# liyheng/MAGPO

Hardware: AMD Instinct MI355X
Metric: env-steps/sec (all agents stepping jointly), CoordSum-4ag, full MAGPO update loop (higher is better)
Workload: dtype f32 (fp32 MFMA; as bf16 x3 operand splits = 24 mantissa bits, six products, fp32 accumulate: the GRU forward scan's recurrent GEMM)

## Files before the change

magpo_amd/csrc/gru.hip:

```cpp
#include "common.hpp"
#include <stdlib.h>

namespace magpo {

constexpr int H = 128;
constexpr int HP = H + LDP;
constexpr int G3 = 3 * H;
constexpr int G3P = G3 + LDP;

struct GruArgs {
  const float* xi;
  const float* Wht;
  const float* b_hn;
  const float* h0;
  const int* h0_idx;
  const unsigned char* reset;
  float* hs;
  float* gates;
  float* hprev;
  int T, A, NR;
  int time_major;
  float* h_last;
  const int* xi_cls;
};

#ifdef MAGPO_GRU_PROF
__device__ unsigned long long g_gru_prof[8];
#define GP_DECL() unsigned long long gp_acc[8] = {0, 0, 0, 0, 0, 0, 0, 0}; unsigned long long gp_last = clock64();
#define GP(k) do { unsigned long long t_ = clock64(); gp_acc[k] += t_ - gp_last; gp_last = t_; } while (0)
#define GP_FLUSH() do { if (threadIdx.x == 0 && (blockIdx.x & 63) == 0) { for (int k_ = 0; k_ < 8; ++k_) atomicAdd(&g_gru_prof[k_], gp_acc[k_]); } } while (0)
#else
#define GP_DECL()
#define GP(k)
#define GP_FLUSH()
#endif

__device__ __forceinline__ long tok_row(int rho, int t, int T, int A) {
  int seq = rho / A, ag = rho - seq * A;
  return ((long)seq * T + t) * A + ag;
}

template <bool FULL, int MODE, int ROWS>
__global__ __launch_bounds__(256, 1) void k_gru_scan_fwd(GruArgs a, int block0) {
  constexpr bool TM = MODE == 1;
  __shared__ __align__(16) float hbuf[2][ROWS * HP];
  extern __shared__ unsigned char rflag[];
  const int tid = threadIdx.x, lane = tid & 63, wave = tid >> 6, lr = lane & 31, h = lane >> 5;
  const int rho0 = (block0 + blockIdx.x) * ROWS;
  const int col = 32 * wave + lr;
  const int T = a.T;
  float4 wf[3][16];
#pragma unroll
  for (int g = 0; g < 3; ++g)
#pragma unroll
    for (int u = 0; u < 16; ++u) wf[g][u] = *reinterpret_cast<const float4*>(a.Wht + ((long)g * H + col) * H + 64 * h + 4 * u);
  const float bhn = a.b_hn[col];
  for (int i = tid; i < ROWS * T; i += 256) {
    const int rl = i / T, t = i - rl * T;
    const int rho = min(rho0 + rl, a.NR - 1);
    rflag[i] = TM ? a.reset[(long)t * (a.NR / a.A) + rho / a.A] : a.reset[(long)(rho / a.A) * T + t];
  }
  int* ctab = reinterpret_cast<int*>(rflag + ROWS * T);
  const bool by_cls = a.xi_cls != nullptr;
  if (by_cls) {
    for (int i = tid; i < ROWS * T; i += 256) {
      const int rl = i / T, t = i - rl * T;
      const int rho = min(rho0 + rl, a.NR - 1);
      ctab[i] = a.xi_cls[TM ? (long)t * a.NR + rho : tok_row(rho, t, T, a.A)];
    }
  }
  for (int i = tid; i < ROWS * (H / 4); i += 256) {
    int r = i / (H / 4), c4 = i - r * (H / 4);
    int rho = rho0 + r;
    float4 v = make_float4(0.f, 0.f, 0.f, 0.f);
    if (rho < a.NR) {
      int seq = rho / a.A;
      if (!(TM ? a.reset[seq] : a.reset[(long)seq * T])) {
        long src = a.h0_idx ? a.h0_idx[rho] : rho;
        v = *reinterpret_cast<const float4*>(a.h0 + src * H + 4 * c4);
      }
    }
    *reinterpret_cast<float4*>(&hbuf[0][r * HP + 4 * c4]) = v;
  }
  __shared__ long rbase[ROWS];
  if (tid < ROWS) rbase[tid] = TM ? (long)min(rho0 + tid, a.NR - 1) : tok_row(min(rho0 + tid, a.NR - 1), 0, T, a.A);
  const long t_stride = TM ? a.NR : a.A;
  __syncthreads();
  GP_DECL();
  for (int t = 0; t < T; ++t) {
    const float* hold = hbuf[t & 1];
    float* hnew = hbuf[(t + 1) & 1];
#pragma unroll
    for (int wr = 0; wr < ROWS / 32; ++wr) {
      GP(6);
      float xr[16], xz[16], xn[16];
      long rowi[16];
#pragma unroll
      for (int i = 0; i < 16; ++i) {
        const int rl = 32 * wr + (i & 3) + 8 * (i >> 2) + 4 * h;
        const long row = rbase[rl] + (long)t * t_stride;
        rowi[i] = row;
        const float* x = a.xi + (by_cls ? (long)ctab[rl * T + t] : row) * G3;
        xr[i] = x[col]; xz[i] = x[H + col]; xn[i] = x[2 * H + col];
      }
      float hpv[16];
      unsigned char rf[16];
      const int tn = t + 1 < T ? t + 1 : t;
#pragma unroll
      for (int i = 0; i < 16; ++i) {
        const int rl = 32 * wr + (i & 3) + 8 * (i >> 2) + 4 * h;
        hpv[i] = hold[rl * HP + col];
        rf[i] = rflag[rl * T + tn];
      }
      GP(0 + 3 * wr);
      f32x16 ar, az, an;
#pragma unroll
      for (int i = 0; i < 16; ++i) { ar[i] = 0.f; az[i] = 0.f; an[i] = 0.f; }
      const float* ap = hold + (32 * wr + lr) * HP + 64 * h;
#pragma unroll
      for (int u = 0; u < 16; ++u) {
        const float4 av = *reinterpret_cast<const float4*>(ap + 4 * u);
        ar = __builtin_amdgcn_mfma_f32_32x32x2f32(av.x, wf[0][u].x, ar, 0, 0, 0);
        az = __builtin_amdgcn_mfma_f32_32x32x2f32(av.x, wf[1][u].x, az, 0, 0, 0);
        an = __builtin_amdgcn_mfma_f32_32x32x2f32(av.x, wf[2][u].x, an, 0, 0, 0);
        ar = __builtin_amdgcn_mfma_f32_32x32x2f32(av.y, wf[0][u].y, ar, 0, 0, 0);
        az = __builtin_amdgcn_mfma_f32_32x32x2f32(av.y, wf[1][u].y, az, 0, 0, 0);
        an = __builtin_amdgcn_mfma_f32_32x32x2f32(av.y, wf[2][u].y, an, 0, 0, 0);
        ar = __builtin_amdgcn_mfma_f32_32x32x2f32(av.z, wf[0][u].z, ar, 0, 0, 0);
        az = __builtin_amdgcn_mfma_f32_32x32x2f32(av.z, wf[1][u].z, az, 0, 0, 0);
        an = __builtin_amdgcn_mfma_f32_32x32x2f32(av.z, wf[2][u].z, an, 0, 0, 0);
        ar = __builtin_amdgcn_mfma_f32_32x32x2f32(av.w, wf[0][u].w, ar, 0, 0, 0);
        az = __builtin_amdgcn_mfma_f32_32x32x2f32(av.w, wf[1][u].w, az, 0, 0, 0);
        an = __builtin_amdgcn_mfma_f32_32x32x2f32(av.w, wf[2][u].w, an, 0, 0, 0);
      }
      GP(1 + 3 * wr);
      const bool more = t + 1 < T;
#pragma unroll
      for (int i = 0; i < 16; ++i) {
        const int rl = 32 * wr + (i & 3) + 8 * (i >> 2) + 4 * h;
        const long row = rowi[i];
        const float hb = an[i] + bhn;
        const float r = fast_sigmoid(xr[i] + ar[i]);
        const float z = fast_sigmoid(xz[i] + az[i]);
        const float n = fast_tanh(xn[i] + r * hb);
        const float hp = hpv[i];
        float hn_new = (1.0f - z) * n + z * hp;
        if (FULL || rho0 + rl < a.NR) {
          if (MODE == 0) {
            a.hs[row * H + col] = hn_new;
            *reinterpret_cast<float4*>(a.gates + row * (4 * H) + 4 * col) = make_float4(r, z, n, hb);
            a.hprev[row * H + col] = hp;
          } else if (MODE == 1) {
            if (!more) a.h_last[(long)(rho0 + rl) * H + col] = hn_new;
          } else {
            if (a.hs) a.hs[row * H + col] = hn_new;
            if (a.gates) {
              *reinterpret_cast<float4*>(a.gates + row * (4 * H) + 4 * col) = make_float4(r, z, n, hb);
            }
            if (a.hprev) a.hprev[row * H + col] = hp;
          }
        }
        hnew[rl * HP + col] = (more & (rf[i] != 0)) ? 0.f : hn_new;
      }
      GP(2 + 3 * wr);
    }
    __syncthreads();
    GP(7);
  }
  GP_FLUSH();
}

constexpr int HB = H + 8;

__device__ __forceinline__ void split_bf16(float x, __bf16& hi, __bf16& lo) {
  hi = (__bf16)x;
  lo = (__bf16)(x - (float)hi);
}

template <bool FULL, int NP>
__global__ __launch_bounds__(256, 1) void k_gru_scan_fwd_bf3(GruArgs a, int block0) {
  constexpr int ROWS = NP == 3 ? 32 : 64;
  __shared__ __align__(16) float hf[ROWS * HP];
  __shared__ __align__(16) __bf16 hsp[2][NP][ROWS * HB];
  extern __shared__ unsigned char rflag[];
  const int tid = threadIdx.x, lane = tid & 63, wave = tid >> 6, lr = lane & 31, h = lane >> 5;
  const int rho0 = (block0 + blockIdx.x) * ROWS;
  const int col = 32 * wave + lr;
  const int T = a.T;
  bf16x8 wp[NP][3][8];
#pragma unroll
  for (int g = 0; g < 3; ++g)
#pragma unroll
    for (int s8 = 0; s8 < 8; ++s8) {
      const float* w = a.Wht + ((long)g * H + col) * H + 64 * h + 8 * s8;
      const float4 w0 = *reinterpret_cast<const float4*>(w), w1 = *reinterpret_cast<const float4*>(w + 4);
      const float wv[8] = {w0.x, w0.y, w0.z, w0.w, w1.x, w1.y, w1.z, w1.w};
#pragma unroll
      for (int j = 0; j < 8; ++j) {
        __bf16 pc[NP];
        split_pieces<NP>(wv[j], pc);
#pragma unroll
        for (int q = 0; q < NP; ++q) wp[q][g][s8][j] = pc[q];
      }
    }
  const float bhn = a.b_hn[col];
  for (int i = tid; i < ROWS * T; i += 256) {
    const int rl = i / T, t = i - rl * T;
    const int rho = min(rho0 + rl, a.NR - 1);
    rflag[i] = a.reset[(long)(rho / a.A) * T + t];
  }
  int* ctab = reinterpret_cast<int*>(rflag + ROWS * T);
  const bool by_cls = a.xi_cls != nullptr;
  if (by_cls) {
    for (int i = tid; i < ROWS * T; i += 256) {
      const int rl = i / T, t = i - rl * T;
      ctab[i] = a.xi_cls[tok_row(min(rho0 + rl, a.NR - 1), t, T, a.A)];
    }
  }
  for (int i = tid; i < ROWS * (H / 4); i += 256) {
    const int r = i / (H / 4), c4 = i - r * (H / 4);
    const int rho = rho0 + r;
    float4 v = make_float4(0.f, 0.f, 0.f, 0.f);
    if (rho < a.NR && !a.reset[(long)(rho / a.A) * T]) {
      const long src = a.h0_idx ? a.h0_idx[rho] : rho;
      v = *reinterpret_cast<const float4*>(a.h0 + src * H + 4 * c4);
    }
    *reinterpret_cast<float4*>(&hf[r * HP + 4 * c4]) = v;
    const float vv[4] = {v.x, v.y, v.z, v.w};
#pragma unroll
    for (int j = 0; j < 4; ++j) {
      __bf16 pc[NP];
      split_pieces<NP>(vv[j], pc);
#pragma unroll
      for (int q = 0; q < NP; ++q) hsp[0][q][r * HB + 4 * c4 + j] = pc[q];
    }
  }
  __shared__ long rbase[ROWS];
  if (tid < ROWS) rbase[tid] = tok_row(min(rho0 + tid, a.NR - 1), 0, T, a.A);
  __syncthreads();
  for (int t = 0; t < T; ++t) {
    const int cur = t & 1, nxt = (t + 1) & 1;
#pragma unroll
// ... 533 lines not shown
```

magpo_amd/csrc/linear.hip:

```cpp
#include "common.hpp"
#include <stdlib.h>

namespace magpo {

enum { ACT_NONE = 0, ACT_RELU = 1, ACT_GELU = 2, ACT_SWISH = 3, ACT_MASKPOS = 4, ACT_TANH = 5, ACT_TANHBWD = 6 };

enum { PRO_EMBED_ACT = 1, PRO_EMBED_OBS = 2, PRO_RESNORM = 3, PRO_HEADMID = 4 };
struct ProArgs {
  const float* a; long lda;
  const float* y; long ldy_;
  const float* s1; const float* s2;
  const float* pe; const int* pos; long pos_stride; int npos; int use_pe;
  const float* W; const int* idx; long idx_stride;
  const float* s_obs; int F;
  float* out; long ldout;
  float* outpe; long ldoutpe;
};

__device__ __forceinline__ float half_row_mean_sq(const float4* v) {
  float s = 0.f;
#pragma unroll
  for (int u = 0; u < 8; ++u) s += v[u].x * v[u].x + v[u].y * v[u].y + v[u].z * v[u].z + v[u].w * v[u].w;
  s += __shfl_xor(s, 32, 64);
  return s * (1.0f / 64.0f);
// ... 364 lines not shown
  const bool do_bias = bias_slab != nullptr && kb == 0;
  const bool full_cols = (c0 + 64 * NB <= NOUT) && ((ldy & 3) == 0);

  WP_DECL();
  if (full_cols) {
    float4 nx[4 + 4 * NB];
    constexpr int YR = 16 * NB;
    const int rx = tid >> 4, cx = 4 * (tid & 15);
    const int ry = tid / YR, cy = 4 * (tid % YR);
    const float* xb = X + kb * 64 + cx;
    const float* yb = dY + c0 + cy;
#define WG_LOADX(J, ROW0) nx[J] = *reinterpret_cast<const float4*>(xb + (long)min((int)(ROW0) + rx + 16 * (J), R - 1) * ldx)
#define WG_LOADY(J, ROW0) nx[4 + (J)] = *reinterpret_cast<const float4*>(yb + (long)min((int)(ROW0) + ry + (256 / YR) * (J), R - 1) * ldy)
    {
      const long row0 = (long)min(g, ntiles - 1) * 64;
#pragma unroll
      for (int j = 0; j < 4; ++j) WG_LOADX(j, row0);
#pragma unroll
      for (int j = 0; j < 4 * NB; ++j) WG_LOADY(j, row0);
    }
    for (int tile = g; tile < ntiles; tile += G) {
      const long row0 = (long)tile * 64;
      const long row0n = (long)min(tile + G, ntiles - 1) * 64;
      __syncthreads();
      WP(0);
#pragma unroll
      for (int j = 0; j < 4; ++j) {
        float4 v = nx[j];
        const bool ok = row0 + rx + 16 * j < R;
        v.x = ok ? v.x : 0.f; v.y = ok ? v.y : 0.f; v.z = ok ? v.z : 0.f; v.w = ok ? v.w : 0.f;
        *reinterpret_cast<float4*>(&xs[(rx + 16 * j) * LDX + cx]) = v;
      }
#pragma unroll
      for (int j = 0; j < 4 * NB; ++j) {
        float4 v = nx[4 + j];
        const bool ok = row0 + ry + (256 / YR) * j < R;
        v.x = ok ? v.x : 0.f; v.y = ok ? v.y : 0.f; v.z = ok ? v.z : 0.f; v.w = ok ? v.w : 0.f;
        *reinterpret_cast<float4*>(&ys[(ry + (256 / YR) * j) * LDY + cy]) = v;
      }
      __syncthreads();
      WP(1);
      WP(2);
#pragma unroll
      for (int s = 0; s < 32; ++s) {
        const int tok = 32 * h + s;
        const float a = xs[tok * LDX + 32 * wr + lr];
#pragma unroll
        for (int b = 0; b < NB; ++b) {
          const float bb = ys[tok * LDY + 64 * b + 32 * wc + lr];
          acc[b] = __builtin_amdgcn_mfma_f32_32x32x2f32(a, bb, acc[b], 0, 0, 0);
        }
        if ((s & 1) && (s >> 1) < 4 + 4 * NB) {
          const int li = s >> 1;
          const float* src = li < 4 ? xb + min(row0n + rx + 16 * li, (long)R - 1) * (long)ldx
                                    : yb + min(row0n + ry + (256 / YR) * (li - 4), (long)R - 1) * (long)ldy;
          nx[li] = *reinterpret_cast<const float4*>(src);
        }
      }
      WP(3);
      if (do_bias && tid < 64 * NB) {
        float sb = 0.f;
#pragma unroll 8
        for (int r = 0; r < 64; ++r) sb += ys[r * LDY + tid];
        bsum += sb;
      }
    }
#undef WG_LOADX
#undef WG_LOADY
  } else {
    float4 xq[4], yq[4 * NB];
    auto fetch = [&](int tile) {
      const long row0 = (long)tile * 64;
  #pragma unroll
      for (int j = 0; j < 4; ++j) {
        const int i = tid + 256 * j;
        const int r = i >> 4, c4 = i & 15;
        const long gr = row0 + r;
        xq[j] = make_float4(0.f, 0.f, 0.f, 0.f);
        if (gr < R) xq[j] = *reinterpret_cast<const float4*>(X + gr * (long)ldx + kb * 64 + 4 * c4);
      }
  #pragma unroll
      for (int j = 0; j < 4 * NB; ++j) {
        const int i = tid + 256 * j;
        const int r = i / (16 * NB), c4 = i - r * (16 * NB);
        const long gr = row0 + r;
        const int col = c0 + 4 * c4;
        float4 v = make_float4(0.f, 0.f, 0.f, 0.f);
        if (gr < R) {
          const float* p = dY + gr * (long)ldy + col;
          if (full_cols || col + 3 < NOUT) v = *reinterpret_cast<const float4*>(p);
          else {
            if (col + 0 < NOUT) v.x = p[0];
            if (col + 1 < NOUT) v.y = p[1];
            if (col + 2 < NOUT) v.z = p[2];
          }
        }
        yq[j] = v;
      }
    };
    auto stash = [&]() {
  #pragma unroll
      for (int j = 0; j < 4; ++j) {
        const int i = tid + 256 * j;
        *reinterpret_cast<float4*>(&xs[(i >> 4) * LDX + 4 * (i & 15)]) = xq[j];
      }
  #pragma unroll
      for (int j = 0; j < 4 * NB; ++j) {
        const int i = tid + 256 * j;
        const int r = i / (16 * NB), c4 = i - r * (16 * NB);
        *reinterpret_cast<float4*>(&ys[r * LDY + 4 * c4]) = yq[j];
      }
    };

    if (g < ntiles) fetch(g);
    for (int tile = g; tile < ntiles; tile += G) {
      __syncthreads();
      stash();
      __syncthreads();
      if (tile + G < ntiles) fetch(tile + G);
#pragma unroll 4
      for (int s = 0; s < 32; ++s) {
        const int tok = 32 * h + s;
        const float a = xs[tok * LDX + 32 * wr + lr];
#pragma unroll
        for (int b = 0; b < NB; ++b) {
          const float bb = ys[tok * LDY + 64 * b + 32 * wc + lr];
          acc[b] = __builtin_amdgcn_mfma_f32_32x32x2f32(a, bb, acc[b], 0, 0, 0);
        }
      }
      if (do_bias && tid < 64 * NB) {
        float sb = 0.f;
#pragma unroll 8
        for (int r = 0; r < 64; ++r) sb += ys[r * LDY + tid];
        bsum += sb;
      }
    }
  }
  WP_FLUSH();
  float* out = slab + (long)g * KIN * NOUT;
#pragma unroll
  for (int b = 0; b < NB; ++b) {
    const int n = c0 + 64 * b + 32 * wc + lr;
    if (n < NOUT) {
#pragma unroll
      for (int i = 0; i < 16; ++i) {
        int kr = kb * 64 + 32 * wr + (i & 3) + 8 * (i >> 2) + 4 * h;
        out[(long)kr * NOUT + n] = acc[b][i];
      }
    }
  }
  if (do_bias && tid < 64 * NB && c0 + tid < NOUT) bias_slab[(long)g * NOUT + c0 + tid] = bsum;
}

__global__ __launch_bounds__(1024) void k_reduce_slabs(const float* __restrict__ slab, float* __restrict__ out, int G, long P, long stride,
                                                       float scale, int accumulate) {
  __shared__ float sh[16][64];
  const int tx = threadIdx.x & 63, ty = threadIdx.x >> 6;
  const long p = (long)blockIdx.x * 64 + tx;
  float s0 = 0.f, s1 = 0.f, s2 = 0.f, s3 = 0.f;
  if (p < P) {
    int g = ty;
    for (; g + 48 < G; g += 64) {
      s0 += slab[(long)g * stride + p];
      s1 += slab[(long)(g + 16) * stride + p];
      s2 += slab[(long)(g + 32) * stride + p];
      s3 += slab[(long)(g + 48) * stride + p];
    }
    for (; g < G; g += 16) s0 += slab[(long)g * stride + p];
  }
  sh[ty][tx] = (s0 + s1) + (s2 + s3);
  __syncthreads();
  if (ty == 0 && p < P) {
    float s = 0.f;
#pragma unroll
    for (int i = 0; i < 16; ++i) s += sh[i][tx];
    s *= scale;
    out[p] = accumulate ? out[p] + s : s;
  }
}

__global__ void k_transpose_pad(const float* __restrict__ W, float* __restrict__ Wt, int K, int N, int Npad) {
  int i = blockIdx.x * blockDim.x + threadIdx.x;
  if (i >= Npad * K) return;
  int n = i / K, k = i - n * K;
  Wt[i] = n < N ? W[(long)k * N + n] : 0.f;
}

template <int KT, int NT>
__global__ __launch_bounds__(256, 1) void k_wgrad_full(const float* __restrict__ X, int ldx, const float* __restrict__ dY, int ldy,
                                                       int R, float* __restrict__ slab, float* __restrict__ bias_slab) {
  constexpr int KIN = 32 * KT, NOUT = 128 * NT, LDX = KIN + LDP, LDY = NOUT + LDP;
  constexpr int NX = 64 * KIN / 4 / 256, NY = 64 * NOUT / 4 / 256;
  extern __shared__ __align__(16) float wf_smem[];
  float* xs = wf_smem;
  float* ys = xs + 64 * LDX;
  const int tid = threadIdx.x, lane = tid & 63, wave = tid >> 6, lr = lane & 31, h = lane >> 5;
  const int g = blockIdx.x, G = gridDim.x;
  const int ntiles = (R + 63) >> 6;
  f32x16 acc[KT][NT];
#pragma unroll
  for (int kt = 0; kt < KT; ++kt)
#pragma unroll
    for (int nt = 0; nt < NT; ++nt)
#pragma unroll
      for (int i = 0; i < 16; ++i) acc[kt][nt][i] = 0.f;
  float bsum[(NOUT + 255) / 256];
#pragma unroll
  for (int j = 0; j < (NOUT + 255) / 256; ++j) bsum[j] = 0.f;
  float4 nx[NX + NY];
#define WF_SRC(LI, ROW0)                                                                                                    \
  ((LI) < NX ? X + min((ROW0) + (tid + 256 * (LI)) / (KIN / 4), (long)R - 1) * (long)ldx + 4 * ((tid + 256 * (LI)) % (KIN / 4)) \
             : dY + min((ROW0) + (tid + 256 * ((LI) - NX)) / (NOUT / 4), (long)R - 1) * (long)ldy + 4 * ((tid + 256 * ((LI) - NX)) % (NOUT / 4)))
  {
    const long row0 = (long)min(g, ntiles - 1) * 64;
#pragma unroll
    for (int li = 0; li < NX + NY; ++li) nx[li] = *reinterpret_cast<const float4*>(WF_SRC(li, row0));
  }
  for (int tile = g; tile < ntiles; tile += G) {
    const long row0 = (long)tile * 64;
    const long row0n = (long)min(tile + G, ntiles - 1) * 64;
    __syncthreads();
#pragma unroll
    for (int li = 0; li < NX + NY; ++li) {
      float4 v = nx[li];
      const int idx = tid + 256 * (li < NX ? li : li - NX);
      const int r = li < NX ? idx / (KIN / 4) : idx / (NOUT / 4);
      const int c = li < NX ? 4 * (idx % (KIN / 4)) : 4 * (idx % (NOUT / 4));
      const bool ok = row0 + r < R;
      v.x = ok ? v.x : 0.f; v.y = ok ? v.y : 0.f; v.z = ok ? v.z : 0.f; v.w = ok ? v.w : 0.f;
      if (li < NX) *reinterpret_cast<float4*>(&xs[r * LDX + c]) = v;
      else *reinterpret_cast<float4*>(&ys[r * LDY + c]) = v;
    }
    __syncthreads();
#pragma unroll
    for (int s = 0; s < 32; ++s) {
      const int tok = 32 * h + s;
      float av[KT], bv[NT];
#pragma unroll
      for (int kt = 0; kt < KT; ++kt) av[kt] = xs[tok * LDX + 32 * kt + lr];
#pragma unroll
      for (int nt = 0; nt < NT; ++nt) bv[nt] = ys[tok * LDY + 32 * NT * wave + 32 * nt + lr];
#pragma unroll
      for (int kt = 0; kt < KT; ++kt)
#pragma unroll
        for (int nt = 0; nt < NT; ++nt) acc[kt][nt] = __builtin_amdgcn_mfma_f32_32x32x2f32(av[kt], bv[nt], acc[kt][nt], 0, 0, 0);
#pragma unroll
      for (int li = 0; li < NX + NY; ++li)
        if (li * 32 / (NX + NY) == s) nx[li] = *reinterpret_cast<const float4*>(WF_SRC(li, row0n));
    }
    if (bias_slab) {
#pragma unroll
      for (int j = 0; j < (NOUT + 255) / 256; ++j) {
        const int col = tid + 256 * j;
        if (col < NOUT) {
          float sb = 0.f;
#pragma unroll 8
          for (int r = 0; r < 64; ++r) sb += ys[r * LDY + col];
          bsum[j] += sb;
        }
      }
    }
  }
#undef WF_SRC
  float* out = slab + (long)g * KIN * NOUT;
#pragma unroll
  for (int kt = 0; kt < KT; ++kt)
#pragma unroll
    for (int nt = 0; nt < NT; ++nt) {
      const int n = 32 * NT * wave + 32 * nt + lr;
#pragma unroll
      for (int i = 0; i < 16; ++i) out[(long)(32 * kt + (i & 3) + 8 * (i >> 2) + 4 * h) * NOUT + n] = acc[kt][nt][i];
    }
  if (bias_slab) {
#pragma unroll
    for (int j = 0; j < (NOUT + 255) / 256; ++j) {
      const int col = tid + 256 * j;
      if (col < NOUT) bias_slab[(long)g * NOUT + col] = bsum[j];
    }
  }
}

__device__ __forceinline__ void split8(const float (&v)[8], bf16x8 (&p)[3]) {
#pragma unroll
  for (int j = 0; j < 8; ++j) {
    __bf16 pc[3];
    split_pieces<3>(v[j], pc);
    p[0][j] = pc[0]; p[1][j] = pc[1]; p[2][j] = pc[2];
  }
}
template <int KT, int NT, int PAD = LDP, bool BF3 = false>
__global__ __launch_bounds__(256, 1) void k_wgrad_full_x(const float* __restrict__ X, int ldx, const float* __restrict__ dY, int ldy,
                                                         int R, float* __restrict__ slab, float* __restrict__ bias_slab) {
  constexpr int KIN = 32 * KT, NOUT = 128 * NT, LDX = KIN + PAD, LDY = NOUT + PAD;
  constexpr int TX = KIN / 4, RPX = 256 / TX, NX = 64 / RPX;
  constexpr int NY = 8 * NT;
  extern __shared__ __align__(16) float wf_smem[];
  float* xs = wf_smem;
  float* ys = xs + 64 * LDX;
  const int tid = threadIdx.x, lane = tid & 63, wave = tid >> 6, lr = lane & 31, h = lane >> 5;
  const int g = blockIdx.x, G = gridDim.x;
  const int ntiles = R >> 6;
  f32x16 acc[KT][NT];
#pragma unroll
  for (int kt = 0; kt < KT; ++kt)
#pragma unroll
    for (int nt = 0; nt < NT; ++nt)
#pragma unroll
      for (int i = 0; i < 16; ++i) acc[kt][nt][i] = 0.f;
  float4 bsum[NT];
#pragma unroll
  for (int j = 0; j < NT; ++j) bsum[j] = make_float4(0.f, 0.f, 0.f, 0.f);
  const unsigned xoff = (unsigned)(tid / TX) * (unsigned)ldx + 4u * (unsigned)(tid % TX);
  const unsigned yoff = (unsigned)(tid >> 5) * (unsigned)ldy + 4u * (unsigned)(tid & 31);
  float* xsw = xs + (tid / TX) * LDX + 4 * (tid % TX);
  float* ysw = ys + (tid >> 5) * LDY + 4 * (tid & 31);
  float4 nxx[NX], nxy[NY];
#define WFX_LOADX(LI, ROW0) nxx[LI] = *reinterpret_cast<const float4*>(X + ((ROW0) + (LI) * RPX) * (long)ldx + xoff)
#define WFX_LOADY(LI, ROW0) nxy[LI] = *reinterpret_cast<const float4*>(dY + ((ROW0) + 8 * ((LI) / NT)) * (long)ldy + 128 * ((LI) % NT) + yoff)
  {
    const long row0 = (long)min(g, ntiles - 1) * 64;
#pragma unroll
    for (int li = 0; li < NX; ++li) { WFX_LOADX(li, row0); }
#pragma unroll
    for (int li = 0; li < NY; ++li) { WFX_LOADY(li, row0); }
  }
  const float* xr = xs + (32 * h) * LDX + lr;
  const float* yr = ys + (32 * h) * LDY + 32 * NT * wave + lr;
  for (int tile = g; tile < ntiles; tile += G) {
    const long row0n = (long)min(tile + G, ntiles - 1) * 64;
    __syncthreads();
#pragma unroll
    for (int li = 0; li < NX; ++li) {
// ... 345 lines not shown
        const float4 a4 = *reinterpret_cast<const float4*>(ard + 4 * u);
        float4 w4;
        if constexpr (WL) w4 = *reinterpret_cast<const float4*>(wrd + 4 * u);
        else w4 = wf[j][u];
        accx = __builtin_amdgcn_mfma_f32_32x32x2f32(a4.x, w4.x, accx, 0, 0, 0);
        accx = __builtin_amdgcn_mfma_f32_32x32x2f32(a4.y, w4.y, accx, 0, 0, 0);
        accx = __builtin_amdgcn_mfma_f32_32x32x2f32(a4.z, w4.z, accx, 0, 0, 0);
        accx = __builtin_amdgcn_mfma_f32_32x32x2f32(a4.w, w4.w, accx, 0, 0, 0);
      }
      const int cb = 32 * (KT * wb + j);
      float* dxt = dX + row0 * lddx + 32 * j;
      const float* mt = MASK == 1 ? aux + row0 * ldaux + 32 * j : nullptr;
#define DB_TR(I) (((I) & 3) + 8 * ((I) >> 2))
      if (full) {
        if constexpr (MASK != 0) {
          float mk[16];
#pragma unroll
          for (int i = 0; i < 16; ++i) mk[i] = MASK == 2 ? xs[(32 * wa + DB_TR(i) + 4 * h) * LDX + cb + lr] : (mt + DB_TR(i) * ldaux)[mo];
#pragma unroll
          for (int i = 0; i < 16; ++i) (dxt + DB_TR(i) * lddx)[so] = mk[i] > 0.f ? accx[i] : 0.f;
        } else {
#pragma unroll
          for (int i = 0; i < 16; ++i) (dxt + DB_TR(i) * lddx)[so] = accx[i];
        }
      } else {
#pragma unroll
        for (int i = 0; i < 16; ++i) {
          if (32 * wa + DB_TR(i) + 4 * h < rleft) {
            float v = accx[i];
            if constexpr (MASK != 0) v = (MASK == 2 ? xs[(32 * wa + DB_TR(i) + 4 * h) * LDX + cb + lr] : (mt + DB_TR(i) * ldaux)[mo]) > 0.f ? v : 0.f;
            (dxt + DB_TR(i) * lddx)[so] = v;
          }
        }
      }
#undef DB_TR
    }
  }
#undef DB_LOADX
#undef DB_LOADY
  if (dwa) {
    const int n = 32 * cbw + lr;
    float* out = slab + (long)g * KIN * NOUT;
    if (n < NOUT) {
#pragma unroll
      for (int kt = 0; kt < KW; ++kt)
#pragma unroll
        for (int i = 0; i < 16; ++i) out[(long)(32 * (kb0 + kt) + (i & 3) + 8 * (i >> 2) + 4 * h) * NOUT + n] = accw[kt][i];
    }
  }
  if (do_bias && bt < NOUT) bias_slab[(long)g * NOUT + bt] = bsum;
}

}

using namespace magpo;

template <auto K>
static auto with_lds(size_t lds) {
  static bool done = false;
  if (!done && lds > 65536) {
    hipFuncSetAttribute(reinterpret_cast<const void*>(K), hipFuncAttributeMaxDynamicSharedMemorySize, (int)lds);
    done = true;
  }
  return K;
}

extern "C" int magpo_linear(const float* X, int ldx, const float* Wt, const float* bias, float* Y, int ldy, float* mask,
                            long R, int KIN, int NOUT, int act, int variant, hipStream_t stream) {
  if (R <= 0) return MAGPO_OK;
  if ((ldx & 3) || NOUT <= 0) { set_error("magpo_linear: ldx must be a multiple of 4, NOUT positive"); return MAGPO_EINVAL; }
  if (KIN != 64 && KIN != 128 && KIN != 192 && KIN != 256 && KIN != 384) { set_error("magpo_linear: KIN must be in {64, 128, 192, 256, 384}"); return MAGPO_EINVAL; }
  if (variant != 0 && variant != 4) { set_error("magpo_linear: variant must be 0 or 4"); return MAGPO_EINVAL; }
  if (act < ACT_NONE || act > ACT_TANHBWD) { set_error("magpo_linear: act must be in [0, 6]"); return MAGPO_EINVAL; }
  const bool needs_mask = act == ACT_MASKPOS || act == ACT_TANHBWD;
  if (needs_mask && !mask) { set_error("magpo_linear: act 4 / 6 (backward masks) need the mask tensor"); return MAGPO_EINVAL; }
  if (!needs_mask && mask) { set_error("magpo_linear: the pre-activation output was removed; the seventh argument is the mask input of act 4 / 6 and must be null otherwise"); return MAGPO_EINVAL; }
  const int ncg = (NOUT + 31) / 32;
  const int nw = (ncg % 4 == 0) ? 4 : 2;
  const int gy = (ncg + nw - 1) / nw;
  const long ntiles = (R + 31) / 32;
  long wk2 = 2048 / nw;
  if (gy >= 3) wk2 /= 2;
  if (wk2 > ntiles) wk2 = ntiles;
  const bool bf3 = variant == 4 && (KIN == 128 || KIN == 192) && nw == 4;
  const size_t lds = bf3 ? (size_t)2 * 3 * 32 * (KIN + 8) * sizeof(__bf16) : (size_t)2 * 32 * (KIN + LDP) * sizeof(float);
  decltype(&k_linear_lds<64, 4>) k;
  if (bf3) k = KIN == 128 ? with_lds<k_linear_lds<128, 4, true>>(lds) : with_lds<k_linear_lds<192, 4, true>>(lds);
  else if (KIN == 64) k = nw == 4 ? with_lds<k_linear_lds<64, 4>>(lds) : with_lds<k_linear_lds<64, 2>>(lds);
  else if (KIN == 128) k = nw == 4 ? with_lds<k_linear_lds<128, 4>>(lds) : with_lds<k_linear_lds<128, 2>>(lds);
  else if (KIN == 192) k = nw == 4 ? with_lds<k_linear_lds<192, 4>>(lds) : with_lds<k_linear_lds<192, 2>>(lds);
  else if (KIN == 256) k = nw == 4 ? with_lds<k_linear_lds<256, 4>>(lds) : with_lds<k_linear_lds<256, 2>>(lds);
  else k = nw == 4 ? with_lds<k_linear_lds<384, 4>>(lds) : with_lds<k_linear_lds<384, 2>>(lds);
  hipLaunchKernelGGL(k, dim3((unsigned)wk2, (unsigned)gy), dim3(64 * nw), lds, stream, X, ldx, Wt, bias, Y, ldy, (int)R, NOUT, act, (const float*)mask);
  return check_launch("magpo_linear");
}

extern "C" int magpo_linear_pro(int pro, const float* a, long lda, const float* y, long ldy_in, const float* s1, const float* s2,
                                const float* pe, const int* pos, long pos_stride, int npos, int use_pe, const float* W,
                                const int* idx, long idx_stride, const float* s_obs, int F, float* out, long ldout,
                                float* outpe, long ldoutpe, const float* Wt, const float* bias, float* Y, long ldy, long R,
                                int NOUT, hipStream_t stream) {
  if (R <= 0) return MAGPO_OK;
  if (pro < 1 || pro > 4 || NOUT <= 0) { set_error("magpo_linear_pro: bad prologue id / NOUT"); return MAGPO_EINVAL; }
  ProArgs p{a, lda, y, ldy_in, s1, s2, pe, pos, pos_stride, npos, use_pe, W, idx, idx_stride, s_obs, F, out, ldout, outpe, ldoutpe};
  const int ncg = (NOUT + 63) / 64;
  const int wpb = ncg < 4 ? ncg : 4;
  const long ntiles = (R + 31) / 32;
  long walkers = 2048 / wpb;
  if (walkers > ntiles) walkers = ntiles;
  dim3 grid((unsigned)walkers, (unsigned)((ncg + 3) / 4)), block(64 * wpb);
#define LP(P_) hipLaunchKernelGGL((k_linear_pro<P_, 2>), grid, block, 0, stream, p, Wt, bias, Y, ldy, (int)R, NOUT)
  switch (pro) {
    case PRO_EMBED_ACT: LP(PRO_EMBED_ACT); break;
    case PRO_EMBED_OBS: LP(PRO_EMBED_OBS); break;
    case PRO_RESNORM: LP(PRO_RESNORM); break;
    default: LP(PRO_HEADMID); break;
  }
#undef LP
  return check_launch("magpo_linear_pro");
}

extern "C" long magpo_wgrad_workspace_floats(int KIN, int NOUT, int G) { return (long)G * ((long)KIN * NOUT + NOUT); }

extern "C" int magpo_wgrad(const float* X, int ldx, const float* dY, int ldy, long R, int KIN, int krows, int NOUT, float* dW,
                           float* db, float* workspace, int G, float scale, int accumulate, int variant, hipStream_t stream) {
  if ((ldx & 3) || (ldy & 3) || KIN % 64) { set_error("magpo_wgrad: bad strides / KIN"); return MAGPO_EINVAL; }
  if (variant != 0 && variant != 64) { set_error("magpo_wgrad: variant must be 0 or 64"); return MAGPO_EINVAL; }
  const bool exact = R % 64 == 0, big = R >= 64 * 256;
  const size_t lds_full = (size_t)64 * (KIN + NOUT) * sizeof(float), lds_pad = (size_t)64 * ((KIN + LDP) + (NOUT + LDP)) * sizeof(float);
  auto bias_slab = [&] { return db ? workspace + (long)G * KIN * NOUT : nullptr; };
  if (big && exact && KIN == 64 && NOUT == 256) {
    if (G > 512) G = 512;
    auto k = with_lds<k_wgrad_full_x<2, 2, 0>>(lds_full);
    hipLaunchKernelGGL(k, dim3(G), dim3(256), lds_full, stream, X, ldx, dY, ldy, (int)R, workspace, bias_slab());
  } else if (big && exact && ((KIN == 64 && NOUT == 192) || (KIN == 128 && NOUT == 128))) {
    if (G > 512) G = 512;
    auto k = KIN == 64 ? with_lds<k_wgrad_full_g<1, 3>>(lds_full) : with_lds<k_wgrad_full_g<2, 2>>(lds_full);
    hipLaunchKernelGGL(k, dim3(G, 1), dim3(256), lds_full, stream, X, ldx, dY, ldy, (int)R, NOUT, workspace, bias_slab());
  } else if (big && KIN == 128 && NOUT == 384) {
    if (G > 256) G = 256;
    auto k = !exact ? with_lds<k_wgrad_full<4, 3>>(lds_pad)
                    : variant == 64 ? with_lds<k_wgrad_full_x<4, 3, LDP, true>>(lds_pad) : with_lds<k_wgrad_full_x<4, 3>>(lds_pad);
    hipLaunchKernelGGL(k, dim3(G), dim3(256), lds_pad, stream, X, ldx, dY, ldy, (int)R, workspace, bias_slab());
  } else {
    const int nb = NOUT >= 128 ? 2 : 1;
    const int per_g = ((NOUT + 64 * nb - 1) / (64 * nb)) * (KIN / 64);
    int g_fit = 256 * (nb == 2 ? 3 : 4) / per_g;
    if (g_fit < 1) g_fit = 1;
    if (G > g_fit) G = g_fit;
    dim3 grid(G, (NOUT + 64 * nb - 1) / (64 * nb), KIN / 64);
    hipLaunchKernelGGL(nb == 2 ? k_wgrad<2> : k_wgrad<1>, grid, dim3(256), 0, stream, X, ldx, dY, ldy, (int)R, KIN, NOUT, workspace, bias_slab());
  }
  const long P = (long)krows * NOUT;
  hipLaunchKernelGGL(k_reduce_slabs, dim3((unsigned)((P + 63) / 64)), dim3(1024), 0, stream, workspace, dW, G, P, (long)KIN * NOUT, scale, accumulate);
  if (db) hipLaunchKernelGGL(k_reduce_slabs, dim3((NOUT + 63) / 64), dim3(1024), 0, stream, bias_slab(), db, G, (long)NOUT, (long)NOUT, scale, accumulate);
  return check_launch("magpo_wgrad");
}

extern "C" int magpo_dense_bwd(const float* X, int ldx, const float* dY, int ldy, const float* W, const float* mask, int ldmask,
                               float* dX, int lddx, long R, int KIN, int NOUT, float* dW, float* db, float* workspace, int G, int act,
                               hipStream_t stream) {
  if (KIN != 64 && KIN != 128) { set_error("magpo_dense_bwd: KIN must be 64 or 128"); return MAGPO_EINVAL; }
  if (NOUT < 1 || NOUT > 64) { set_error("magpo_dense_bwd: NOUT must be in [1, 64]"); return MAGPO_EINVAL; }
  if ((ldx & 3) || (ldy & 3) || (lddx & 3) || ldx < KIN || lddx < KIN || ldy < NOUT) {
    set_error("magpo_dense_bwd: ldx, ldy, lddx must be multiples of 4 and cover KIN / NOUT / KIN columns"); return MAGPO_EINVAL;
  }
  if (act != ACT_NONE && act != ACT_MASKPOS) { set_error("magpo_dense_bwd: act must be 0 or 4"); return MAGPO_EINVAL; }
  if (act == ACT_MASKPOS && !mask) { set_error("magpo_dense_bwd: act 4 needs the mask tensor"); return MAGPO_EINVAL; }
  if (act == ACT_NONE && mask) { set_error("magpo_dense_bwd: the mask argument must be null for act 0"); return MAGPO_EINVAL; }
  if (mask && ((ldmask & 3) || ldmask < KIN)) { set_error("magpo_dense_bwd: ldmask must be a multiple of 4 and cover KIN columns"); return MAGPO_EINVAL; }
  if (R < 1 || R > 0x7fffffffL - 64 || G < 1) { set_error("magpo_dense_bwd: R must be in [1, 2^31 - 65], G positive"); return MAGPO_EINVAL; }
  if (((uintptr_t)X | (uintptr_t)dY) & 15) { set_error("magpo_dense_bwd: X and dY must be 16-byte aligned"); return MAGPO_EINVAL; }
  if (G > 512) G = 512;
  if (G > (R + 63) / 64) G = (int)((R + 63) / 64);
  float* bias_slab = db ? workspace + (long)G * KIN * NOUT : nullptr;
  const int m = act != ACT_MASKPOS ? 0 : (mask == X && ldmask == ldx) ? 2 : 1;
  const bool k2 = KIN == 128, n2 = NOUT > 32;
  decltype(&k_dense_bwd<1, 1, 0>) k;
#define DB_PICK(KT_, NT_) (m == 0 ? k_dense_bwd<KT_, NT_, 0> : m == 1 ? k_dense_bwd<KT_, NT_, 1> : k_dense_bwd<KT_, NT_, 2>)
  if (!k2 && !n2) k = DB_PICK(1, 1);
  else if (!k2) k = DB_PICK(1, 2);
  else if (!n2) k = DB_PICK(2, 1);
  else k = DB_PICK(2, 2);
#undef DB_PICK
  hipLaunchKernelGGL(k, dim3(G), dim3(256), 0, stream, X, ldx, dY, ldy, W, mask, ldmask, dX, lddx, (int)R, NOUT, workspace, bias_slab);
  const long P = (long)KIN * NOUT;
  hipLaunchKernelGGL(k_reduce_slabs, dim3((unsigned)((P + 63) / 64)), dim3(1024), 0, stream, workspace, dW, G, P, P, 1.0f, 0);
  if (db) hipLaunchKernelGGL(k_reduce_slabs, dim3(1), dim3(1024), 0, stream, bias_slab, db, G, (long)NOUT, (long)NOUT, 1.0f, 0);
  return check_launch("magpo_dense_bwd");
}

extern "C" int magpo_reduce_slabs(const float* slab, float* out, int G, long P, long stride, float scale, int accumulate, hipStream_t stream) {
  hipLaunchKernelGGL(k_reduce_slabs, dim3((unsigned)((P + 63) / 64)), dim3(1024), 0, stream, slab, out, G, P, stride, scale, accumulate);
  return check_launch("magpo_reduce_slabs");
}

extern "C" int magpo_transpose_pad(const float* W, float* Wt, int K, int N, int Npad, hipStream_t stream) {
  int total = Npad * K;
  hipLaunchKernelGGL(k_transpose_pad, dim3((total + 255) / 256), dim3(256), 0, stream, W, Wt, K, N, Npad);
  return check_launch("magpo_transpose_pad");
}

#ifdef MAGPO_WG_PROF
extern "C" int magpo_debug_wg_prof(unsigned long long* out_host, int reset) {
  if (hipMemcpyFromSymbol(out_host, HIP_SYMBOL(magpo::g_wg_prof), sizeof(unsigned long long) * 8) != hipSuccess) return MAGPO_ELAUNCH;
  if (reset) { unsigned long long z[8] = {0}; if (hipMemcpyToSymbol(HIP_SYMBOL(magpo::g_wg_prof), z, sizeof(z)) != hipSuccess) return MAGPO_ELAUNCH; }
  return MAGPO_OK;
}
#endif
```

Measured before the change: 4.232 million.

## Skip GRU scan steps before last reset; batch slab reductions into one launch

```diff
diff --git a/magpo_amd/csrc/gru.hip b/magpo_amd/csrc/gru.hip
--- a/magpo_amd/csrc/gru.hip
+++ b/magpo_amd/csrc/gru.hip
@@ -55,10 +55,19 @@
 #pragma unroll
     for (int u = 0; u < 16; ++u) wf[g][u] = *reinterpret_cast<const float4*>(a.Wht + ((long)g * H + col) * H + 64 * h + 4 * u);
   const float bhn = a.b_hn[col];
+  __shared__ __align__(16) int last[TM ? ROWS : 4];
+  if constexpr (TM) {
+    if (tid < ROWS) last[tid] = 0;
+    __syncthreads();
+  }
   for (int i = tid; i < ROWS * T; i += 256) {
     const int rl = i / T, t = i - rl * T;
     const int rho = min(rho0 + rl, a.NR - 1);
-    rflag[i] = TM ? a.reset[(long)t * (a.NR / a.A) + rho / a.A] : a.reset[(long)(rho / a.A) * T + t];
+    const unsigned char f = TM ? a.reset[(long)t * (a.NR / a.A) + rho / a.A] : a.reset[(long)(rho / a.A) * T + t];
+    rflag[i] = f;
+    if constexpr (TM) {
+      if (f && t > 0) atomicMax(&last[rl], t);
+    }
   }
   int* ctab = reinterpret_cast<int*>(rflag + ROWS * T);
   const bool by_cls = a.xi_cls != nullptr;
@@ -69,25 +78,36 @@
       ctab[i] = a.xi_cls[TM ? (long)t * a.NR + rho : tok_row(rho, t, T, a.A)];
     }
   }
+  int t0 = 0;
+  if constexpr (TM) {
+    __syncthreads();
+    int m = T;
+#pragma unroll
+    for (int r4 = 0; r4 < ROWS / 4; ++r4) {
+      const int4 l4 = *reinterpret_cast<const int4*>(&last[4 * r4]);
+      m = min(min(m, min(l4.x, l4.y)), min(l4.z, l4.w));
+    }
+    t0 = __builtin_amdgcn_readfirstlane(m);
+  }
   for (int i = tid; i < ROWS * (H / 4); i += 256) {
     int r = i / (H / 4), c4 = i - r * (H / 4);
     int rho = rho0 + r;
     float4 v = make_float4(0.f, 0.f, 0.f, 0.f);
-    if (rho < a.NR) {
+    if (rho < a.NR && t0 == 0) {
       int seq = rho / a.A;
       if (!(TM ? a.reset[seq] : a.reset[(long)seq * T])) {
         long src = a.h0_idx ? a.h0_idx[rho] : rho;
         v = *reinterpret_cast<const float4*>(a.h0 + src * H + 4 * c4);
       }
     }
-    *reinterpret_cast<float4*>(&hbuf[0][r * HP + 4 * c4]) = v;
+    *reinterpret_cast<float4*>(&hbuf[t0 & 1][r * HP + 4 * c4]) = v;
   }
   __shared__ long rbase[ROWS];
   if (tid < ROWS) rbase[tid] = TM ? (long)min(rho0 + tid, a.NR - 1) : tok_row(min(rho0 + tid, a.NR - 1), 0, T, a.A);
   const long t_stride = TM ? a.NR : a.A;
   __syncthreads();
   GP_DECL();
-  for (int t = 0; t < T; ++t) {
+  for (int t = t0; t < T; ++t) {
     const float* hold = hbuf[t & 1];
     float* hnew = hbuf[(t + 1) & 1];
 #pragma unroll
diff --git a/magpo_amd/csrc/linear.hip b/magpo_amd/csrc/linear.hip
--- a/magpo_amd/csrc/linear.hip
+++ b/magpo_amd/csrc/linear.hip
@@ -540,14 +540,26 @@
   if (do_bias && tid < 64 * NB && c0 + tid < NOUT) bias_slab[(long)g * NOUT + c0 + tid] = bsum;
 }
 
-__global__ __launch_bounds__(1024) void k_reduce_slabs(const float* __restrict__ slab, float* __restrict__ out, int G, long P, long stride,
-                                                       float scale, int accumulate) {
+__device__ __forceinline__ void fold_block(const float* __restrict__ slab, float* __restrict__ out, int G, long P, long stride, float scale,
+                                           int accumulate, long block) {
   __shared__ float sh[16][64];
   const int tx = threadIdx.x & 63, ty = threadIdx.x >> 6;
-  const long p = (long)blockIdx.x * 64 + tx;
+  const long p = block * 64 + tx;
   float s0 = 0.f, s1 = 0.f, s2 = 0.f, s3 = 0.f;
   if (p < P) {
     int g = ty;
+    for (; g + 240 < G; g += 256) {
+      float v[16];
+#pragma unroll
+      for (int k = 0; k < 16; ++k) v[k] = slab[(long)(g + 16 * k) * stride + p];
+#pragma unroll
+      for (int k = 0; k < 16; k += 4) {
+        s0 += v[k];
+        s1 += v[k + 1];
+        s2 += v[k + 2];
+        s3 += v[k + 3];
+      }
+    }
     for (; g + 48 < G; g += 64) {
       s0 += slab[(long)g * stride + p];
       s1 += slab[(long)(g + 16) * stride + p];
@@ -566,6 +578,51 @@
     out[p] = accumulate ? out[p] + s : s;
   }
 }
+
+__global__ __launch_bounds__(1024) void k_reduce_slabs(const float* __restrict__ slab, float* __restrict__ out, int G, long P, long stride,
+                                                       float scale, int accumulate) {
+  fold_block(slab, out, G, P, stride, scale, accumulate, blockIdx.x);
+}
+
+struct FoldJob {
+  const float* slab;
+  float* out;
+  long P, stride;
+  int G, accumulate;
+  float scale;
+};
+struct FoldJobs {
+  FoldJob job[4];
+  unsigned first[5];
+};
+
+__global__ __launch_bounds__(1024) void k_reduce_slabs_multi(FoldJobs t) {
+  const unsigned b = blockIdx.x;
+  const int j = (b >= t.first[1]) + (b >= t.first[2]) + (b >= t.first[3]);
+  const FoldJob& f = t.job[j];
+  fold_block(f.slab, f.out, f.G, f.P, f.stride, f.scale, f.accumulate, b - t.first[j]);
+}
+
+struct FoldLaunch {
+  FoldJobs t{};
+  int n = 0;
+  void add(const float* slab, float* out, int G, long P, long stride, float scale, int accumulate) {
+    if (P <= 0) return;
+    t.job[n] = FoldJob{slab, out, P, stride, G, accumulate, scale};
+    t.first[n + 1] = t.first[n] + (unsigned)((P + 63) / 64);
+    ++n;
+  }
+  void launch(hipStream_t stream) {
+    if (n == 0) return;
+    if (n == 1) {
+      const FoldJob& f = t.job[0];
+      hipLaunchKernelGGL(k_reduce_slabs, dim3(t.first[1]), dim3(1024), 0, stream, f.slab, f.out, f.G, f.P, f.stride, f.scale, f.accumulate);
+      return;
+    }
+    for (int j = n; j < 4; ++j) t.first[j + 1] = 0xffffffffu;
+    hipLaunchKernelGGL(k_reduce_slabs_multi, dim3(t.first[n]), dim3(1024), 0, stream, t);
+  }
+};
 
 __global__ void k_transpose_pad(const float* __restrict__ W, float* __restrict__ Wt, int K, int N, int Npad) {
   int i = blockIdx.x * blockDim.x + threadIdx.x;
@@ -1217,8 +1274,10 @@
     hipLaunchKernelGGL(nb == 2 ? k_wgrad<2> : k_wgrad<1>, grid, dim3(256), 0, stream, X, ldx, dY, ldy, (int)R, KIN, NOUT, workspace, bias_slab());
   }
   const long P = (long)krows * NOUT;
-  hipLaunchKernelGGL(k_reduce_slabs, dim3((unsigned)((P + 63) / 64)), dim3(1024), 0, stream, workspace, dW, G, P, (long)KIN * NOUT, scale, accumulate);
-  if (db) hipLaunchKernelGGL(k_reduce_slabs, dim3((NOUT + 63) / 64), dim3(1024), 0, stream, bias_slab(), db, G, (long)NOUT, (long)NOUT, scale, accumulate);
+  FoldLaunch folds;
+  folds.add(workspace, dW, G, P, (long)KIN * NOUT, scale, accumulate);
+  if (db) folds.add(bias_slab(), db, G, (long)NOUT, (long)NOUT, scale, accumulate);
+  folds.launch(stream);
   return check_launch("magpo_wgrad");
 }
 
@@ -1250,8 +1309,10 @@
 #undef DB_PICK
   hipLaunchKernelGGL(k, dim3(G), dim3(256), 0, stream, X, ldx, dY, ldy, W, mask, ldmask, dX, lddx, (int)R, NOUT, workspace, bias_slab);
   const long P = (long)KIN * NOUT;
-  hipLaunchKernelGGL(k_reduce_slabs, dim3((unsigned)((P + 63) / 64)), dim3(1024), 0, stream, workspace, dW, G, P, P, 1.0f, 0);
-  if (db) hipLaunchKernelGGL(k_reduce_slabs, dim3(1), dim3(1024), 0, stream, bias_slab, db, G, (long)NOUT, (long)NOUT, 1.0f, 0);
+  FoldLaunch folds;
+  folds.add(workspace, dW, G, P, P, 1.0f, 0);
+  if (db) folds.add(bias_slab, db, G, (long)NOUT, (long)NOUT, 1.0f, 0);
+  folds.launch(stream);
   return check_launch("magpo_dense_bwd");
 }
 
```

Measured after the change: 4.272 million (median of 6 runs). No clear change (+0.9%).
